# achraf-15/neural_image_compression

Measured on AMD Instinct MI355X. Metric: images/sec (256x256 RGB, batch 32) fwd+bwd, higher is better.
Workload: dtype f32; 1 GPU; cfg2: JointAutoregressiveHierarchical(M=192,K=1) fwd+rd_loss(lambda=0.01)+bwd+Adam, 32x3x256x256 per GPU, fp32; global_batch=32, parallelism=dp1, step=eager (autograd)

## Files before the change

### include/lic.h

```cpp
#ifndef LIC_H
#define LIC_H

#include <stddef.h>
#include <stdint.h>

#ifdef __cplusplus
extern "C" {
#endif

#define LIC_ABI_VERSION 4

typedef void* lic_stream_t;

enum lic_status {
  LIC_OK = 0,
  LIC_ERR_INVALID = -1,
  LIC_ERR_UNSUPPORTED = -2,
  LIC_ERR_LAUNCH = -3,
  LIC_ERR_WORKSPACE = -4
};

enum lic_epilogue {
  LIC_EPI_NONE = 0,
  LIC_EPI_LEAKY = 1,
// ... 256 lines not shown
                 double bias_correction2, lic_stream_t stream);

enum { LIC_REDUCE_SLABS = 0, LIC_REDUCE_COLUMNS = 1 };
enum { LIC_REDUCE_EPI_NONE = 0, LIC_REDUCE_EPI_REPARAM = 1 };
#define LIC_REDUCE_MAX_JOBS 32
typedef struct lic_reduce_job {
  const float* src;
  float* dst;
  const float* param;
  int64_t sm, smr, sn, snr, stap;
  int32_t kind, epilogue;
  int32_t splitk, ntaps, Cm, Cn, Mvalid, Nvalid, mdiv, ndiv;
  float scale, bound;
  int32_t block0, nblocks;
} lic_reduce_job;
int lic_wgrad_bf16_partial(const lic_wgrad_desc* d, void* workspace, size_t workspace_bytes, lic_reduce_job* job,
                           lic_stream_t stream);
int lic_colsum_bf16_partial(const void* in, int64_t ld, int64_t P, int32_t C, float scale, float* out, void* workspace,
                            size_t workspace_bytes, lic_reduce_job* job, lic_stream_t stream);
int lic_colsum2_bf16_partial(const void* in_a, const void* in_b, int64_t ld, int64_t P, int32_t C, float scale,
                             float* out_a, float* out_b, void* workspace, size_t workspace_bytes, lic_reduce_job* jobs2,
                             lic_stream_t stream);
int lic_leaky_bwd_colsum_bf16(const void* y, const void* dy, void* dx, int64_t P, int32_t C, float slope, float* out,
                              void* workspace, size_t workspace_bytes, lic_reduce_job* job, lic_stream_t stream);
int lic_reduce_batch(const lic_reduce_job* jobs, int32_t njobs, lic_stream_t stream);

int lic_head_convt_bf16_supported(int32_t Cin, int32_t Cout, int32_t kh, int32_t kw, int32_t stride, int32_t pad,
                                  int32_t out_pad);
int lic_head_convt_bf16(const void* x, const void* w_packed, const float* bias, float* out, int32_t B, int32_t Hi,
                        int32_t Wi, int32_t Cin, lic_stream_t stream);
int lic_stem_conv_bf16(const float* x, const void* w_packed, const float* bias, void* y, int32_t B, int32_t H, int32_t W,
                       int32_t Cout, lic_stream_t stream);

typedef struct lic_plan lic_plan;
int lic_plan_create(void* hip_graph, lic_plan** out);
int lic_plan_info(const lic_plan* plan, int64_t* info);
int lic_plan_replay(lic_plan* plan, lic_stream_t main, const lic_stream_t* sides, int32_t n_sides);
int lic_plan_tune(lic_plan* plan, lic_stream_t main, const lic_stream_t* sides, int32_t n_sides, double* result);
void lic_plan_destroy(lic_plan* plan);
const char* lic_plan_last_error(void);

int lic_version(void);
int lic_last_hip_error(void);
const char* lic_arch(void);

#ifdef __cplusplus
}
#endif
#endif
```

### neural_image_compression_amd/_lib.py

```python
from __future__ import annotations

import ctypes as C
import os

_HERE = os.path.dirname(os.path.abspath(__file__))
LIB_PATH = os.path.join(_HERE, "liblic_hip.so")

EPI_NONE, EPI_LEAKY, EPI_MUL_LEAKY_MASK, EPI_GDN, EPI_IGDN, EPI_GDN_BWD, EPI_IGDN_BWD, EPI_CONV_GDN, EPI_CONV_IGDN = range(9)
FE_NPARAM = 43

_vp, _i32, _i64, _f32, _sz = C.c_void_p, C.c_int32, C.c_int64, C.c_float, C.c_size_t


class IgemmDesc(C.Structure):
    _fields_ = [("in_", _vp), ("w", _vp), ("bias", _vp), ("out", _vp), ("out2", _vp), ("aux", _vp),
                ("aux2", _vp), ("aux3", _vp), ("res", _vp),
                ("in_ld", _i64), ("out_ld", _i64), ("out2_ld", _i64), ("aux_ld", _i64),
                ("aux2_ld", _i64), ("aux3_ld", _i64), ("res_ld", _i64),
                ("B", _i32), ("Hi", _i32), ("Wi", _i32), ("Cin", _i32),
                ("Ho", _i32), ("Wo", _i32), ("Cout", _i32),
                ("kh", _i32), ("kw", _i32), ("stride", _i32), ("pad", _i32),
                ("transposed", _i32), ("prologue", _i32), ("epilogue", _i32),
                ("tap_mask", C.c_uint32), ("slope", _f32), ("workspace", _vp), ("workspace_bytes", _sz),
                ("out3", _vp), ("out3_ld", _i64),
# ... 118 lines not shown
    "lic_gdn_bwd_bf16_partial_rows": (_i64, [_i64]),
    "lic_gdn_bwd_bf16": (C.c_int, [_vp, _vp, _vp, _vp, _vp, _vp, _vp, _vp, _i64, _i32, _i32, _vp]),
    "lic_gdn_bwd_bf16_recompute": (C.c_int, [_vp, _vp, _vp, _vp, _vp, _vp, _vp, _vp, _vp, _i64, _i32, _i32, _vp]),
    "lic_leaky_bwd_bf16": (C.c_int, [_vp, _vp, _vp, _i64, _f32, _vp]),
    "lic_leaky_bwd_colsum_bf16": (C.c_int, [_vp, _vp, _vp, _i64, _i32, _f32, _vp, _vp, _sz, C.POINTER(ReduceJob), _vp]),
    "lic_igemm_fused_gdn_supported": (C.c_int, [_i32, _i32]),
    "lic_igemm_fused_gdn_preferred": (C.c_int, [C.POINTER(IgemmDesc)]),
    "lic_gdn_supported": (C.c_int, [_i32]),
    "lic_gdn_fwd": (C.c_int, [_vp, _vp, _vp, _vp, _vp, _vp, _i64, _i32, _i32, _vp]),
    "lic_gdn_bwd_partial_rows": (_i64, [_i64]),
    "lic_gdn_bwd": (C.c_int, [_vp, _vp, _vp, _vp, _vp, _vp, _vp, _vp, _i64, _i32, _i32, _vp]),
    "lic_factorized_cdf_tables": (C.c_int, [_vp, _i32, _i32, _i32, _vp, _vp]),
    "lic_gmm_cdf_tables": (C.c_int, [_vp, _i64, _i32, _i32, _i32, _vp, _vp, _vp]),
    "lic_rans_decode_step": (C.c_int, [_vp] * 8 + [_i32] * 4 + [_vp, _vp, _i64, _vp]),
    "lic_rans_encode_pick": (C.c_int, [_vp] * 4 + [_i32, _i64, _i32, _i32] + [_vp] * 4),
    "lic_rans_encode": (C.c_int, [_vp] * 3 + [_i64, _i32, _i64, _vp, _i64, _vp, _vp, _vp]),
    "lic_msssim_workspace_bytes": (_sz, [_i32, _i32, _i32, _i32]),
    "lic_msssim": (C.c_int, [_vp, _vp, _i32, _i32, _i32, _i32, _i64, _i64, _i64, _i64, _f32, _vp, _vp, _vp, _sz,
                             _vp]),
    "lic_msssim_bwd_workspace_bytes": (_sz, [_i32, _i32, _i32, _i32]),
    "lic_msssim_bwd": (C.c_int, [_vp, _vp, _i32, _i32, _i32, _i32, _i64, _i64, _i64, _i64, _f32, _vp, _vp, _sz, _vp,
                                 _vp, _vp, _sz, _vp]),
    "lic_u8_to_f32": (C.c_int, [_vp, _vp, _i64, _vp]),
    "lic_window_u8_to_f32": (C.c_int, [_vp, _vp, _i32, _i32, _i32, _i32, _i32, _vp, _vp]),
    "lic_window_f32": (C.c_int, [_vp, _i64, _i64, _i64, _i64] + [_i32] * 9 + [_vp, _vp]),
    "lic_tensor_stats_workspace_bytes": (_sz, []),
    "lic_tensor_stats": (C.c_int, [_vp, _i64, _i32, _f32, _f32, _vp, _vp, _vp, _sz, _vp]),
    "lic_prep_plan": (_i64, [C.POINTER(PrepJob), _i32]),
    "lic_prep_run": (C.c_int, [_vp, _i32, _i64, _vp]),
    "lic_adam_plan": (_i64, [C.POINTER(AdamJob), _i32]),
    "lic_adam_run": (C.c_int, [_vp, _i32, _i64, _vp] + [C.c_double] * 7 + [_vp]),
    "lic_head_convt_bf16_supported": (C.c_int, [_i32] * 7),
    "lic_head_convt_bf16": (C.c_int, [_vp, _vp, _vp, _vp, _i32, _i32, _i32, _i32, _vp]),
    "lic_stem_conv_bf16": (C.c_int, [_vp, _vp, _vp, _vp, _i32, _i32, _i32, _i32, _vp]),
    "lic_plan_create": (C.c_int, [_vp, C.POINTER(C.c_void_p)]),
    "lic_plan_info": (C.c_int, [_vp, C.POINTER(C.c_int64)]),
    "lic_plan_replay": (C.c_int, [_vp, _vp, C.POINTER(C.c_void_p), _i32]),
    "lic_plan_tune": (C.c_int, [_vp, _vp, C.POINTER(C.c_void_p), _i32, C.POINTER(C.c_double)]),
    "lic_plan_destroy": (None, [_vp]),
    "lic_plan_last_error": (C.c_char_p, []),
    "lic_version": (C.c_int, []),
    "lic_last_hip_error": (C.c_int, []),
    "lic_arch": (C.c_char_p, []),
}

_lib = None


class LicError(RuntimeError):
    pass


def load():
    global _lib
    if _lib is None:
        if not os.path.exists(LIB_PATH):
            raise LicError(
                f"{LIB_PATH} not found: the HIP extension is not built. Run "
                "`python -c 'import __graft_entry__ as g; g.build()'` (or make -C "
                "neural_image_compression_amd/csrc). There is no CPU fallback.")
        lib = C.CDLL(LIB_PATH)
        for name, (res, args) in SIGNATURES.items():
            fn = getattr(lib, name)
            fn.restype = res
            fn.argtypes = args
        _lib = lib
    return _lib
# ... 10 lines not shown
```

### neural_image_compression_amd/functional.py

```python
from __future__ import annotations

import ctypes as C
from typing import Optional, Tuple

import torch

from . import _lib as L
from .reductions import can_defer, defer, flush_point, flush_reductions

PEDESTAL = float(2.0 ** -36)
LIKELIHOOD_BOUND = 1e-9

PROFILE = None
PROFILE_MIN_FLOP = 0.0
FORCE_IGEMM = None
FORCE_WGRAD = None
KERNEL_TRACE = None
GRAD_VIEWS = {}
PREPARED = {}
AUX_STREAM = None
PLAN_RECORDING = False


_raw_stream = getattr(torch._C, "_cuda_getCurrentRawStream", None)
# ... 332 lines not shown
    return _pack_conv_weight(weight.detach(), False, for_dgrad=False)


@torch.no_grad()
def conv2d_prepacked(x, w_packed, bias, cout, kernel, stride=1, padding=0, leaky=False, slope=0.01, tap_mask=0,
                     pin_tile=False):
    _require_cuda(x, w_packed, bias)
    xh = _nhwc(x)
    B, Hi, Wi, Cin = xh.shape
    Ho, Wo = conv_out_size(Hi, Wi, kernel, stride, padding, False)
    out = torch.empty((B, Ho, Wo, cout), device=x.device, dtype=torch.float32)
    global FORCE_IGEMM
    saved = FORCE_IGEMM
    if pin_tile and Cin % 4 == 0 and cout % 64 == 0:
        FORCE_IGEMM = (64, 1, 0)
    try:
        _igemm(xh, w_packed, out, B=B, Hi=Hi, Wi=Wi, Cin=Cin, Ho=Ho, Wo=Wo, Cout=cout, kh=kernel, kw=kernel,
               stride=stride, pad=padding, transposed=False, bias=bias,
               epilogue=L.EPI_LEAKY if leaky else L.EPI_NONE, slope=slope, tap_mask=tap_mask)
    finally:
        FORCE_IGEMM = saved
    return _nchw_view(out)


def conv_transpose2d(x, weight, bias, stride=1, padding=0, output_padding=0, leaky=False, slope=0.01,
                     residual=None):
    return _ConvFn.apply(x, weight, bias, stride, padding, output_padding, True, leaky, slope, 0, residual)


def _kpad(kh, kw, c):
    return (kh * kw * c + 3) // 4 * 4


def _image_conv_columns(xh, weight, stride, pad):
    B, Hi, Wi, Cin = xh.shape
    Cout, _, kh, kw = weight.shape
    Ho, Wo = conv_out_size(Hi, Wi, kh, stride, pad, False)
    Kp = _kpad(kh, kw, Cin)
    P = B * Ho * Wo
    col = torch.empty((P, Kp), device=xh.device, dtype=torch.float32)
    L.check(L.load().lic_im2col(_ptr(xh), _ptr(col), B, Hi, Wi, Cin, Ho, Wo, kh, kw, stride, pad, Kp,
                                _stream()), "lic_im2col")
    taps = kh * kw
    wpk = prepared(weight, "f32.stem")
    if wpk is None:
        wp = torch.zeros((Kp, Cout), device=xh.device, dtype=torch.float32)
        _permute3(weight.contiguous(), wp, (taps, Cin, Cout), (1, taps, Cin * taps), (Cin * Cout, Cout, 1))
        wpk = _pack_dense(wp)
    return col, wpk, Ho, Wo, Kp


def _image_conv_backward(col, weight, g, stride, pad, in_shape, need_dx, need_dw, need_db):
    B, Hi, Wi, Cin = in_shape
    _, Ho, Wo, Cout = g.shape
    _, _, kh, kw = weight.shape
    taps, Kp, P = kh * kw, col.shape[1], B * Ho * Wo
    lib = L.load()
    dx = dw = db = None
    if need_dx:
        wpT = torch.zeros((Cout, Kp), device=g.device, dtype=torch.float32)
        _permute3(weight.contiguous(), wpT, (Cout, Cin, taps), (Cin * taps, taps, 1), (Kp, 1, Cin))
        dcol = torch.empty((P, Kp), device=g.device, dtype=torch.float32)
        _igemm(g, _pack_dense(wpT), dcol, B=1, Hi=1, Wi=P, Cin=Cout, Ho=1, Wo=P, Cout=Kp, kh=1, kw=1, stride=1,
               pad=0, transposed=False)
        dxh = torch.empty((B, Hi, Wi, Cin), device=g.device, dtype=torch.float32)
        L.check(lib.lic_col2im(_ptr(dcol), None, _ptr(dxh), B, Ho, Wo, Cin, Hi, Wi, kh, kw, stride,
                               pad, Kp, _stream()), "lic_col2im")
        dx = _nchw_view(dxh)
    if need_dw:
        dw = grad_like(weight)
        tmp = torch.empty((Kp, Cout), device=g.device, dtype=torch.float32)
        _wgrad(col, g, tmp, B=1, Hs=1, Ws=P, Cp=Kp, Hl=1, Wl=P, Cg=Cout, kh=1, kw=1, stride=1, pad=0,
               g_is_row=False, dst_sm=Cout, dst_sn=1, dst_stap=0)
        _permute3(tmp, dw, (taps, Cin, Cout), (Cin * Cout, Cout, 1), (1, taps, Cin * taps))
    if need_db:
        db = _bias_grad(g, P, Cout)
    return dx, dw, db


class _ImageConvFn(torch.autograd.Function):

    @staticmethod
    def forward(ctx, x, weight, bias, stride, pad, leaky, slope):
        _require_cuda(x, weight, bias)
        xh = _nhwc(x)
        B = xh.shape[0]
        Cout = weight.shape[0]
        col, wp, Ho, Wo, Kp = _image_conv_columns(xh, weight, stride, pad)
        P = B * Ho * Wo
        out = torch.empty((B, Ho, Wo, Cout), device=x.device, dtype=torch.float32)
        _igemm(col, wp, out, B=1, Hi=1, Wi=P, Cin=Kp, Ho=1, Wo=P, Cout=Cout, kh=1, kw=1, stride=1,
               pad=0, transposed=False, bias=bias, epilogue=L.EPI_LEAKY if leaky else L.EPI_NONE,
               slope=slope)
        ctx.save_for_backward(col, weight, out if leaky else None)
        ctx.cfg = (stride, pad, leaky, slope, tuple(xh.shape), bias is not None)
        return _nchw_view(out)

    @staticmethod
    def backward(ctx, gy):
        col, weight, yh = ctx.saved_tensors
        stride, pad, leaky, slope, in_shape, has_bias = ctx.cfg
        g = _nhwc(gy)
        if leaky:
            g = _leaky_bwd(yh, g, slope)
        else:
            _carry_partial(gy, g)
        dx, dw, db = _image_conv_backward(col, weight, g, stride, pad, in_shape, ctx.needs_input_grad[0],
                                          ctx.needs_input_grad[1], has_bias and ctx.needs_input_grad[2])
        return dx, dw, db, None, None, None, None


class _ImageConvGDNFn(torch.autograd.Function):

    @staticmethod
    def forward(ctx, x, weight, bias, beta, gamma, stride, pad, inverse, beta_bound, gamma_bound, pedestal, keep=True):
        _require_cuda(x, weight, bias, beta, gamma)
        xh = _nhwc(x)
        B = xh.shape[0]
        Cout = weight.shape[0]
        col, wp, Ho, Wo, Kp = _image_conv_columns(xh, weight, stride, pad)
        P = B * Ho * Wo
        beta_e, gT = _gdn_operands(beta, gamma, beta_bound, gamma_bound, pedestal)
        y = torch.empty((B, Ho, Wo, Cout), device=x.device, dtype=torch.float32)
        conv_out = torch.empty_like(y) if keep else None
        norm = torch.empty_like(y) if keep else None
        _igemm(col, wp, y, B=1, Hi=1, Wi=P, Cin=Kp, Ho=1, Wo=P, Cout=Cout, kh=1, kw=1, stride=1,
               pad=0, transposed=False, bias=bias, epilogue=L.EPI_CONV_IGDN if inverse else L.EPI_CONV_GDN,
               out2=norm, out3=conv_out, aux=gT, aux2=beta_e)
        ctx.save_for_backward(col, weight, conv_out, norm, beta, gamma)
        ctx.cfg = (stride, pad, tuple(xh.shape), inverse, beta_bound, gamma_bound, bias is not None, pedestal)
        return _nchw_view(y)

    @staticmethod
    def backward(ctx, gy):
        col, weight, conv_out, norm, beta, gamma = ctx.saved_tensors
        stride, pad, in_shape, inverse, beta_bound, gamma_bound, has_bias, pedestal = ctx.cfg
        need = ctx.needs_input_grad
        g_conv, dbeta, dgamma = _gdn_backward(conv_out, norm, beta, gamma, _nhwc(gy), inverse,
                                              beta_bound, gamma_bound, pedestal, True, need[3], need[4])
        dx, dw, db = _image_conv_backward(col, weight, g_conv, stride, pad, in_shape, need[0], need[1],
                                          has_bias and need[2])
        return dx, dw, db, dbeta, dgamma, None, None, None, None, None, None, None


class _ImageConvTFn(torch.autograd.Function):

    @staticmethod
    def forward(ctx, x, weight, bias, stride, pad, out_pad):
        _require_cuda(x, weight, bias)
        xh = _nhwc(x)
        B, Hi, Wi, Cin = xh.shape
        _, Cout, kh, kw = weight.shape
        Ho, Wo = conv_out_size(Hi, Wi, kh, stride, pad, True, out_pad)
        taps, Kp, P = kh * kw, _kpad(kh, kw, Cout), B * Hi * Wi
        lib = L.load()
        wpk = prepared(weight, "f32.head")
        if wpk is None:
            wp = torch.zeros((Cin, Kp), device=x.device, dtype=torch.float32)
            _permute3(weight.contiguous(), wp, (Cin, Cout, taps), (Cout * taps, taps, 1), (Kp, 1, Cout))
            wpk = _pack_dense(wp)
        col = torch.empty((P, Kp), device=x.device, dtype=torch.float32)
        _igemm(xh, wpk, col, B=1, Hi=1, Wi=P, Cin=Cin, Ho=1, Wo=P, Cout=Kp, kh=1, kw=1, stride=1, pad=0,
               transposed=False)
        out = torch.empty((B, Ho, Wo, Cout), device=x.device, dtype=torch.float32)
        L.check(lib.lic_col2im(_ptr(col), _ptr(bias), _ptr(out), B, Hi, Wi, Cout, Ho, Wo, kh, kw, stride,
                               pad, Kp, _stream()), "lic_col2im")
        ctx.save_for_backward(xh, weight)
        ctx.cfg = (stride, pad, (Ho, Wo), bias is not None)
        return _nchw_view(out)

    @staticmethod
    def backward(ctx, gy):
        xh, weight = ctx.saved_tensors
        stride, pad, (Ho, Wo), has_bias = ctx.cfg
        g = _nhwc(gy)
        B, Hi, Wi, Cin = xh.shape
        _, Cout, kh, kw = weight.shape
        taps, Kp, P = kh * kw, _kpad(kh, kw, Cout), B * Hi * Wi
        lib = L.load()
        dcol = torch.empty((P, Kp), device=g.device, dtype=torch.float32)
        L.check(lib.lic_im2col(_ptr(g), _ptr(dcol), B, Ho, Wo, Cout, Hi, Wi, kh, kw, stride, pad, Kp,
                               _stream()), "lic_im2col")
        dx = dw = db = None
        if ctx.needs_input_grad[0]:
            wpk = prepared(weight, "f32.head_dx")
            if wpk is None:
                wpT = torch.zeros((Kp, Cin), device=g.device, dtype=torch.float32)
                _permute3(weight.contiguous(), wpT, (taps, Cout, Cin), (1, taps, Cout * taps),
                          (Cout * Cin, Cin, 1))
                wpk = _pack_dense(wpT)
            dxh = torch.empty_like(xh)
            _igemm(dcol, wpk, dxh, B=1, Hi=1, Wi=P, Cin=Kp, Ho=1, Wo=P, Cout=Cin, kh=1, kw=1, stride=1,
                   pad=0, transposed=False)
            dx = _nchw_view(dxh)
        if ctx.needs_input_grad[1]:
            dw = grad_like(weight)
            tmp = torch.empty((Cin, Kp), device=g.device, dtype=torch.float32)
            _wgrad(xh, dcol, tmp, B=1, Hs=1, Ws=P, Cp=Cin, Hl=1, Wl=P, Cg=Kp, kh=1, kw=1, stride=1, pad=0,
                   g_is_row=True, dst_sm=1, dst_sn=Kp, dst_stap=0)
            _permute3(tmp, dw, (Cin, taps, Cout), (Kp, Cout, 1), (Cout * taps, 1, taps))
        if has_bias and ctx.needs_input_grad[2]:
            db = _colsum(g, B * Ho * Wo, Cout)
        return dx, dw, db, None, None, None


def image_conv2d(x, weight, bias, stride, padding, leaky=False, slope=0.01):
    return _ImageConvFn.apply(x, weight, bias, stride, padding, leaky, slope)


def image_conv_transpose2d(x, weight, bias, stride, padding, output_padding):
    return _ImageConvTFn.apply(x, weight, bias, stride, padding, output_padding)


class _LeakyFn(torch.autograd.Function):
    @staticmethod
    def forward(ctx, x, slope):
        _require_cuda(x)
        xc = x.contiguous()
        y = _leaky_bwd(xc, xc, slope)
        ctx.save_for_backward(y)
        ctx.slope = slope
        return y

    @staticmethod
    def backward(ctx, gy):
        (y,) = ctx.saved_tensors
        return _leaky_bwd(y, gy.contiguous(), ctx.slope), None


def leaky_relu(x, slope=0.01):
    return _LeakyFn.apply(x, slope)


class _GDNFn(torch.autograd.Function):
    @staticmethod
    def forward(ctx, x, beta, gamma, inverse, beta_bound, gamma_bound, pedestal, res, keep=True):
# ... 562 lines not shown
```

Measured before the change: 1433 images/s.

## Add fused f32 MFMA kernel for the 3-channel transposed-conv image head

Adds a direct HIP kernel for the stride-2 5x5 transposed convolution that produces the RGB output. Each block computes a halo tile's per-tap partial products with f32 MFMA into shared memory, then gathers them into output pixels with the bias added. This replaces the igemm into a padded column buffer followed by a separate col2im pass, so the large intermediate column tensor is no longer written and re-read. Only the forward path changes; the backward still uses the existing col-based route, and the shape restrictions fall back to the old path otherwise.

```diff
diff --git a/include/lic.h b/include/lic.h
--- a/include/lic.h
+++ b/include/lic.h
@@ -312,6 +312,11 @@
 int lic_stem_conv_bf16(const float* x, const void* w_packed, const float* bias, void* y, int32_t B, int32_t H, int32_t W,
                        int32_t Cout, lic_stream_t stream);
 
+int lic_head_convt_f32_supported(int32_t Cin, int32_t Cout, int32_t kh, int32_t kw, int32_t stride, int32_t pad,
+                                 int32_t out_pad);
+int lic_head_convt_f32(const float* x, const float* w, const float* bias, float* out, int32_t B, int32_t Hi, int32_t Wi,
+                       int32_t Cin, lic_stream_t stream);
+
 typedef struct lic_plan lic_plan;
 int lic_plan_create(void* hip_graph, lic_plan** out);
 int lic_plan_info(const lic_plan* plan, int64_t* info);
diff --git a/neural_image_compression_amd/_lib.py b/neural_image_compression_amd/_lib.py
--- a/neural_image_compression_amd/_lib.py
+++ b/neural_image_compression_amd/_lib.py
@@ -174,6 +174,8 @@
     "lic_adam_run": (C.c_int, [_vp, _i32, _i64, _vp] + [C.c_double] * 7 + [_vp]),
     "lic_head_convt_bf16_supported": (C.c_int, [_i32] * 7),
     "lic_head_convt_bf16": (C.c_int, [_vp, _vp, _vp, _vp, _i32, _i32, _i32, _i32, _vp]),
+    "lic_head_convt_f32_supported": (C.c_int, [_i32] * 7),
+    "lic_head_convt_f32": (C.c_int, [_vp, _vp, _vp, _vp, _i32, _i32, _i32, _i32, _vp]),
     "lic_stem_conv_bf16": (C.c_int, [_vp, _vp, _vp, _vp, _i32, _i32, _i32, _i32, _vp]),
     "lic_plan_create": (C.c_int, [_vp, C.POINTER(C.c_void_p)]),
     "lic_plan_info": (C.c_int, [_vp, C.POINTER(C.c_int64)]),
diff --git a/neural_image_compression_amd/csrc/lic_head_f32.hip b/neural_image_compression_amd/csrc/lic_head_f32.hip
--- /dev/null
+++ b/neural_image_compression_amd/csrc/lic_head_f32.hip
@@ -0,0 +1,172 @@
+#include "lic_common.h"
+
+namespace {
+
+constexpr int HF_TH = 8, HF_TW = 16;
+constexpr int HF_HR = HF_TH + 2, HF_HC = HF_TW + 2;
+constexpr int HF_HP = HF_HR * HF_HC;
+constexpr int HF_PT = 3;
+constexpr int HF_LD = 84;
+constexpr int HF_NT = 5;
+static_assert(4 * HF_PT * 16 >= HF_HP, "the four waves cover the halo block");
+
+struct HeadF32Params {
+  const float* x;
+  const float* w;
+  const float* bias;
+  float* out;
+  int B, Hi, Wi, tiles_x, tiles_y;
+  long ntiles;
+};
+
+template <int NC>
+__global__ __launch_bounds__(256) void head_convt_f32_kernel(const HeadF32Params p) {
+  constexpr int C = 16 * NC, WLD = C + 4;
+  __shared__ __attribute__((aligned(16))) float wl[16 * HF_NT * WLD];
+  __shared__ __attribute__((aligned(16))) float col[4 * HF_PT * 16 * HF_LD];
+  const int tid = threadIdx.x, lane = tid & 63, l16 = lane & 15, g = lane >> 4;
+  const int wave = __builtin_amdgcn_readfirstlane(tid >> 6);
+  for (int i = tid; i < 5 * WLD; i += 256) wl[75 * WLD + i] = 0.0f;
+  for (int i = tid; i < C * 75; i += 256) {
+    const int ci = i / 75, r = i - ci * 75, co = r / 25, tap = r - co * 25;
+    wl[(3 * tap + co) * WLD + ci] = p.w[i];
+  }
+  float bs[3] = {0.f, 0.f, 0.f};
+  if (p.bias)
+#pragma unroll
+    for (int c = 0; c < 3; ++c) bs[c] = p.bias[c];
+  const int Ho = 2 * p.Hi, Wo = 2 * p.Wi;
+  __syncthreads();
+
+  for (long tile = blockIdx.x; tile < p.ntiles; tile += gridDim.x) {
+    const int tx = (int)(tile % p.tiles_x);
+    const long rest = tile / p.tiles_x;
+    const int ty = (int)(rest % p.tiles_y), b = (int)(rest / p.tiles_y);
+    const int y0 = ty * HF_TH, x0 = tx * HF_TW;
+    const float* src[HF_PT];
+    bool ok[HF_PT];
+#pragma unroll
+    for (int i = 0; i < HF_PT; ++i) {
+      const int hp = (wave * HF_PT + i) * 16 + l16;
+      const int hr = hp / HF_HC, hc = hp - hr * HF_HC;
+      const int iy = y0 - 1 + hr, ix = x0 - 1 + hc;
+      ok[i] = hp < HF_HP && iy >= 0 && iy < p.Hi && ix >= 0 && ix < p.Wi;
+      src[i] = p.x + (((long)b * p.Hi + (ok[i] ? iy : 0)) * p.Wi + (ok[i] ? ix : 0)) * C + 4 * g;
+    }
+    f32x4 acc[HF_PT][HF_NT];
+#pragma unroll
+    for (int i = 0; i < HF_PT; ++i)
+#pragma unroll
+      for (int t = 0; t < HF_NT; ++t) acc[i][t] = f32x4{0.f, 0.f, 0.f, 0.f};
+    f32x4 xq[HF_PT], xn[HF_PT];
+#pragma unroll
+    for (int i = 0; i < HF_PT; ++i) xq[i] = *reinterpret_cast<const f32x4*>(src[i]);
+#pragma unroll
+    for (int c = 0; c < NC; ++c) {
+      if (c + 1 < NC)
+#pragma unroll
+        for (int i = 0; i < HF_PT; ++i) xn[i] = *reinterpret_cast<const f32x4*>(src[i] + 16 * (c + 1));
+      f32x4 wf[HF_NT];
+#pragma unroll
+      for (int t = 0; t < HF_NT; ++t) wf[t] = *reinterpret_cast<const f32x4*>(wl + (16 * t + l16) * WLD + 16 * c + 4 * g);
+#pragma unroll
+      for (int i = 0; i < HF_PT; ++i)
+        if (!ok[i]) xq[i] = f32x4{0.f, 0.f, 0.f, 0.f};
+#pragma unroll
+      for (int e = 0; e < 4; ++e)
+#pragma unroll
+        for (int t = 0; t < HF_NT; ++t)
+#pragma unroll
+          for (int i = 0; i < HF_PT; ++i)
+            acc[i][t] = __builtin_amdgcn_mfma_f32_16x16x4f32(wf[t][e], xq[i][e], acc[i][t], 0, 0, 0);
+#pragma unroll
+      for (int i = 0; i < HF_PT; ++i) xq[i] = xn[i];
+    }
+#pragma unroll
+    for (int i = 0; i < HF_PT; ++i) {
+      float* row = col + ((wave * HF_PT + i) * 16 + l16) * HF_LD + 4 * g;
+#pragma unroll
+      for (int t = 0; t < HF_NT; ++t) *reinterpret_cast<f32x4*>(row + 16 * t) = acc[i][t];
+    }
+    __syncthreads();
+#pragma unroll
+    for (int h = 0; h < 2; ++h) {
+      const int oyl = (tid >> 5) + 8 * h, oxl = tid & 31;
+      const int qy = oyl >> 1, py = oyl & 1, qx = oxl >> 1, px = oxl & 1;
+      float o0 = bs[0], o1 = bs[1], o2 = bs[2];
+#pragma unroll
+      for (int a = 0; a < 3; ++a) {
+        const int ky = py + 2 * a;
+        if (ky > 4) continue;
+        const int hr = qy + 2 - a;
+#pragma unroll
+        for (int bb = 0; bb < 3; ++bb) {
+          const int kx = px + 2 * bb;
+          if (kx > 4) continue;
+          const int hc = qx + 2 - bb;
+          const float* c3 = col + (hr * HF_HC + hc) * HF_LD + 3 * (5 * ky + kx);
+          o0 += c3[0];
+          o1 += c3[1];
+          o2 += c3[2];
+        }
+      }
+      const int oy = 2 * y0 + oyl, ox = 2 * x0 + oxl;
+      if (oy < Ho && ox < Wo) {
+        float* dst = p.out + (((long)b * Ho + oy) * Wo + ox) * 3;
+        dst[0] = o0;
+        dst[1] = o1;
+        dst[2] = o2;
+      }
+    }
+    __syncthreads();
+  }
+}
+
+template <int NC>
+int head_f32_launch(const HeadF32Params& p, hipStream_t s) {
+  static const int slots = [] {
+    int per_cu = 0, cus = 0, devid = 0;
+    if (hipOccupancyMaxActiveBlocksPerMultiprocessor(&per_cu, (const void*)head_convt_f32_kernel<NC>, 256, 0) != hipSuccess || per_cu < 1)
+      per_cu = 1;
+    if (hipGetDevice(&devid) != hipSuccess ||
+        hipDeviceGetAttribute(&cus, hipDeviceAttributeMultiprocessorCount, devid) != hipSuccess || cus < 1)
+      cus = 256;
+    return per_cu * cus;
+  }();
+  long grid = p.ntiles < slots ? p.ntiles : slots;
+  const long rounds = (p.ntiles + grid - 1) / grid;
+  grid = (p.ntiles + rounds - 1) / rounds;
+  hipLaunchKernelGGL((head_convt_f32_kernel<NC>), dim3((unsigned)grid), dim3(256), 0, s, p);
+  return lic_check_launch();
+}
+
+}
+
+LIC_EXPORT int lic_head_convt_f32_supported(int32_t Cin, int32_t Cout, int32_t kh, int32_t kw, int32_t stride, int32_t pad,
+                                            int32_t out_pad) {
+  return (Cin == 64 || Cin == 128 || Cin == 192) && Cout == 3 && kh == 5 && kw == 5 && stride == 2 && pad == 2 && out_pad == 1;
+}
+
+LIC_EXPORT int lic_head_convt_f32(const float* x, const float* w, const float* bias, float* out, int32_t B, int32_t Hi,
+                                  int32_t Wi, int32_t Cin, lic_stream_t stream) {
+  if (!x || !w || !out || B <= 0 || Hi <= 0 || Wi <= 0) return LIC_ERR_INVALID;
+  if (!(Cin == 64 || Cin == 128 || Cin == 192)) return LIC_ERR_UNSUPPORTED;
+  if ((reinterpret_cast<uintptr_t>(x) & 15) || (reinterpret_cast<uintptr_t>(w) & 3) || (reinterpret_cast<uintptr_t>(out) & 3))
+    return LIC_ERR_INVALID;
+  HeadF32Params p;
+  p.x = x;
+  p.w = w;
+  p.bias = bias;
+  p.out = out;
+  p.B = B;
+  p.Hi = Hi;
+  p.Wi = Wi;
+  p.tiles_x = (Wi + HF_TW - 1) / HF_TW;
+  p.tiles_y = (Hi + HF_TH - 1) / HF_TH;
+  p.ntiles = (long)B * p.tiles_x * p.tiles_y;
+  if ((long)B * Hi * Wi * Cin > 0x7FFFFFFFFFL) return LIC_ERR_UNSUPPORTED;
+  hipStream_t s = (hipStream_t)stream;
+  if (Cin == 64) return head_f32_launch<4>(p, s);
+  if (Cin == 128) return head_f32_launch<8>(p, s);
+  return head_f32_launch<12>(p, s);
+}
diff --git a/neural_image_compression_amd/functional.py b/neural_image_compression_amd/functional.py
--- a/neural_image_compression_amd/functional.py
+++ b/neural_image_compression_amd/functional.py
@@ -510,6 +510,17 @@
         Ho, Wo = conv_out_size(Hi, Wi, kh, stride, pad, True, out_pad)
         taps, Kp, P = kh * kw, _kpad(kh, kw, Cout), B * Hi * Wi
         lib = L.load()
+        if head_direct_supported(Cin, Cout, kh, kw, stride, pad, out_pad):
+            out = torch.empty((B, Ho, Wo, Cout), device=x.device, dtype=torch.float32)
+            wc = weight.contiguous()
+            name = f"head_convt_f32_kernel<{Cin // 16}>"
+            _trace(name)
+            _timed(name, 2.0 * P * Cin * taps * Cout, 4 * (P * Cin + B * Ho * Wo * Cout),
+                   lambda: L.check(lib.lic_head_convt_f32(_ptr(xh), _ptr(wc), _ptr(bias), _ptr(out), B, Hi, Wi, Cin,
+                                                          _stream()), "lic_head_convt_f32"))
+            ctx.save_for_backward(xh, weight)
+            ctx.cfg = (stride, pad, (Ho, Wo), bias is not None)
+            return _nchw_view(out)
         wpk = prepared(weight, "f32.head")
         if wpk is None:
             wp = torch.zeros((Cin, Kp), device=x.device, dtype=torch.float32)
@@ -558,6 +569,10 @@
         if has_bias and ctx.needs_input_grad[2]:
             db = _colsum(g, B * Ho * Wo, Cout)
         return dx, dw, db, None, None, None
+
+
+def head_direct_supported(Cin, Cout, kh, kw, stride, pad, out_pad) -> bool:
+    return bool(L.load().lic_head_convt_f32_supported(Cin, Cout, kh, kw, stride, pad, out_pad))
 
 
 def image_conv2d(x, weight, bias, stride, padding, leaky=False, slope=0.01):
```

Result: no change. 1439 images/s, median of 6 (+0.4%).

## Add direct fp32 RGB stem/head conv kernels avoiding im2col/col2im buffers

Applied to the files above, without the earlier changes.

Adds HIP kernels for the 5x5 stride-2 RGB convolutions: a transposed-conv head that computes per-tile columns in LDS and scatters them directly, a stem-style conv for its input gradient, and a patch weight-gradient kernel that builds image patches in LDS. These replace the large materialised im2col/col2im column buffers and their separate GEMMs. The image-conv forward now saves the raw input instead of the column matrix for backward. This cuts global memory traffic and buffer allocation, but adds fixed-shape kernels and a split-K slab reduction.

```diff
diff --git a/include/lic.h b/include/lic.h
--- a/include/lic.h
+++ b/include/lic.h
@@ -312,6 +312,15 @@
 int lic_stem_conv_bf16(const float* x, const void* w_packed, const float* bias, void* y, int32_t B, int32_t H, int32_t W,
                        int32_t Cout, lic_stream_t stream);
 
+int lic_rgb_f32_supported(int32_t C, int32_t Crgb, int32_t kh, int32_t kw, int32_t stride, int32_t pad);
+int lic_head_convt_f32(const float* x, const float* w_packed, const float* bias, float* out, int32_t B, int32_t Hi,
+                       int32_t Wi, int32_t Cin, lic_stream_t stream);
+int lic_stem_conv_f32(const float* x, const float* w_packed, float* y, int32_t B, int32_t H, int32_t W, int32_t Cout,
+                      lic_stream_t stream);
+size_t lic_patch_wgrad_f32_workspace_bytes(int32_t B, int32_t H, int32_t W, int32_t C);
+int lic_patch_wgrad_f32(const float* img, const float* act, float* dst, int32_t B, int32_t H, int32_t W, int32_t C,
+                        int64_t dst_sm, int64_t dst_sn, void* workspace, size_t workspace_bytes, lic_stream_t stream);
+
 typedef struct lic_plan lic_plan;
 int lic_plan_create(void* hip_graph, lic_plan** out);
 int lic_plan_info(const lic_plan* plan, int64_t* info);
diff --git a/neural_image_compression_amd/_lib.py b/neural_image_compression_amd/_lib.py
--- a/neural_image_compression_amd/_lib.py
+++ b/neural_image_compression_amd/_lib.py
@@ -175,6 +175,11 @@
     "lic_head_convt_bf16_supported": (C.c_int, [_i32] * 7),
     "lic_head_convt_bf16": (C.c_int, [_vp, _vp, _vp, _vp, _i32, _i32, _i32, _i32, _vp]),
     "lic_stem_conv_bf16": (C.c_int, [_vp, _vp, _vp, _vp, _i32, _i32, _i32, _i32, _vp]),
+    "lic_rgb_f32_supported": (C.c_int, [_i32] * 6),
+    "lic_head_convt_f32": (C.c_int, [_vp, _vp, _vp, _vp, _i32, _i32, _i32, _i32, _vp]),
+    "lic_stem_conv_f32": (C.c_int, [_vp, _vp, _vp, _i32, _i32, _i32, _i32, _vp]),
+    "lic_patch_wgrad_f32_workspace_bytes": (_sz, [_i32] * 4),
+    "lic_patch_wgrad_f32": (C.c_int, [_vp, _vp, _vp, _i32, _i32, _i32, _i32, _i64, _i64, _vp, _sz, _vp]),
     "lic_plan_create": (C.c_int, [_vp, C.POINTER(C.c_void_p)]),
     "lic_plan_info": (C.c_int, [_vp, C.POINTER(C.c_int64)]),
     "lic_plan_replay": (C.c_int, [_vp, _vp, C.POINTER(C.c_void_p), _i32]),
diff --git a/neural_image_compression_amd/csrc/lic_rgb_f32.hip b/neural_image_compression_amd/csrc/lic_rgb_f32.hip
--- /dev/null
+++ b/neural_image_compression_amd/csrc/lic_rgb_f32.hip
@@ -0,0 +1,440 @@
+#include "lic_common.h"
+#include "lic_conv_plan.h"
+
+namespace {
+
+constexpr int RG_TH = 8, RG_TW = 16;
+constexpr int RG_HR = RG_TH + 2, RG_HC = RG_TW + 2;
+constexpr int RG_HP = RG_HR * RG_HC;
+constexpr int RG_MT = (RG_HP + 15) / 16;
+constexpr int RG_LD = 84;
+constexpr int RG_IR = 2 * RG_TH + 3, RG_IC = 2 * RG_TW + 3;
+constexpr int RG_IMG = RG_IR * RG_IC * 3;
+constexpr int RG_K = 75, RG_KP = 76, RG_KT = 5;
+
+__device__ __forceinline__ long rg_pk(int k, int n, int ntile) {
+  const int cb = k >> 4, r = k & 15;
+  return ((((long)cb * ntile + (n >> 5)) * 2 + ((r >> 2) & 1)) * 64 + ((r >> 3) << 5) + (n & 31)) * 4 + (r & 3);
+}
+
+__device__ __forceinline__ void rg_panel_to_lds(const float* __restrict__ w, float* lds, int K4, int N, int ntile) {
+  for (int i = threadIdx.x; i < K4 * N; i += 256) {
+    const int k4 = i / N, n = i - k4 * N;
+    *reinterpret_cast<f32x4*>(lds + 4 * i) = *reinterpret_cast<const f32x4*>(w + rg_pk(4 * k4, n, ntile));
+  }
+}
+
+__device__ __forceinline__ void rg_image_to_lds(const float* __restrict__ img, float* lds, int b, int H, int W, int y0, int x0) {
+  for (int i = threadIdx.x; i < RG_IMG; i += 256) {
+    const int r = i / (RG_IC * 3), c3 = i - r * (RG_IC * 3);
+    const int iy = 2 * y0 - 2 + r, ix = 2 * x0 - 2 + c3 / 3;
+    float v = 0.0f;
+    if (iy >= 0 && iy < H && ix >= 0 && ix < W) v = img[(((long)b * H + iy) * W + ix) * 3 + (c3 % 3)];
+    lds[i] = v;
+  }
+}
+
+__device__ __forceinline__ int rg_col_ofs(int kc) {
+  const int tap = kc / 3, co = kc - 3 * tap;
+  const int ky = tap / 5, kx = tap - 5 * ky;
+  return (ky * RG_IC + kx) * 3 + co;
+}
+
+struct TileGeom {
+  int tiles_x, tiles_y;
+  long ntiles;
+};
+
+struct HeadParams {
+  const float* x;
+  const float* w;
+  const float* bias;
+  float* out;
+  int B, Hi, Wi;
+  TileGeom g;
+};
+
+template <int NC>
+__global__ __launch_bounds__(256, 1) void head_convt_f32_kernel(const HeadParams p) {
+  constexpr int C = 16 * NC;
+  __shared__ __attribute__((aligned(16))) float wl[C * 80];
+  __shared__ __attribute__((aligned(16))) float col[RG_MT * 16 * RG_LD];
+  const int tid = threadIdx.x, lane = tid & 63, li = lane & 15, kq = lane >> 4;
+  const int wave = __builtin_amdgcn_readfirstlane(tid >> 6);
+  rg_panel_to_lds(p.w, wl, C / 4, 80, 4);
+  float bs[3] = {0.f, 0.f, 0.f};
+  if (p.bias)
+#pragma unroll
+    for (int c = 0; c < 3; ++c) bs[c] = p.bias[c];
+  const int Ho = 2 * p.Hi, Wo = 2 * p.Wi;
+  __syncthreads();
+
+  for (long tile = blockIdx.x; tile < p.g.ntiles; tile += gridDim.x) {
+    const int tx = (int)(tile % p.g.tiles_x);
+    const long rest = tile / p.g.tiles_x;
+    const int ty = (int)(rest % p.g.tiles_y), b = (int)(rest / p.g.tiles_y);
+    const int y0 = ty * RG_TH, x0 = tx * RG_TW;
+    f32x4 xq[2][NC];
+    auto load = [&](int m, f32x4* dst) {
+      const int hp = m * 16 + li;
+      const int hr = hp / RG_HC, hc = hp - hr * RG_HC;
+      const int iy = y0 - 1 + hr, ix = x0 - 1 + hc;
+      const bool ok = hp < RG_HP && iy >= 0 && iy < p.Hi && ix >= 0 && ix < p.Wi;
+      const float* src = p.x + (((long)b * p.Hi + (ok ? iy : 0)) * p.Wi + (ok ? ix : 0)) * C + 4 * kq;
+#pragma unroll
+      for (int q = 0; q < NC; ++q) dst[q] = *reinterpret_cast<const f32x4*>(src + 16 * q);
+      if (!ok)
+#pragma unroll
+        for (int q = 0; q < NC; ++q) dst[q] = f32x4{0.f, 0.f, 0.f, 0.f};
+    };
+    load(wave, xq[0]);
+#pragma unroll
+    for (int it = 0; it < RG_MT / 4; ++it) {
+      const int m = wave + 4 * it;
+      if (it + 1 < RG_MT / 4) load(m + 4, xq[(it + 1) & 1]);
+      const f32x4* xv = xq[it & 1];
+      f32x4 acc[RG_KT];
+#pragma unroll
+      for (int t = 0; t < RG_KT; ++t) acc[t] = f32x4{0.f, 0.f, 0.f, 0.f};
+#pragma unroll
+      for (int q = 0; q < NC; ++q) {
+#pragma unroll
+        for (int t = 0; t < RG_KT; ++t) {
+          const f32x4 wv = *reinterpret_cast<const f32x4*>(wl + ((q * 4 + kq) * 80 + 16 * t + li) * 4);
+#pragma unroll
+          for (int j = 0; j < 4; ++j) acc[t] = __builtin_amdgcn_mfma_f32_16x16x4f32(wv[j], xv[q][j], acc[t], 0, 0, 0);
+        }
+      }
+      float* row = col + (m * 16 + li) * RG_LD + 4 * kq;
+#pragma unroll
+      for (int t = 0; t < RG_KT; ++t) *reinterpret_cast<f32x4*>(row + 16 * t) = acc[t];
+    }
+    __syncthreads();
+#pragma unroll
+    for (int h = 0; h < 2; ++h) {
+      const int oyl = (tid >> 5) + 8 * h, oxl = tid & 31;
+      const int qy = oyl >> 1, py = oyl & 1, qx = oxl >> 1, px = oxl & 1;
+      float o0 = bs[0], o1 = bs[1], o2 = bs[2];
+#pragma unroll
+      for (int a = 0; a < 3; ++a) {
+        const int ky = py + 2 * a;
+        if (ky > 4) continue;
+        const int hr = qy + 2 - a;
+#pragma unroll
+        for (int bb = 0; bb < 3; ++bb) {
+          const int kx = px + 2 * bb;
+          if (kx > 4) continue;
+          const int hc = qx + 2 - bb;
+          const float* c3 = col + (hr * RG_HC + hc) * RG_LD + 3 * (5 * ky + kx);
+          o0 += c3[0];
+          o1 += c3[1];
+          o2 += c3[2];
+        }
+      }
+      const int oy = 2 * y0 + oyl, ox = 2 * x0 + oxl;
+      if (oy < Ho && ox < Wo) {
+        float* dst = p.out + (((long)b * Ho + oy) * Wo + ox) * 3;
+        dst[0] = o0;
+        dst[1] = o1;
+        dst[2] = o2;
+      }
+    }
+    __syncthreads();
+  }
+}
+
+struct StemParams {
+  const float* x;
+  const float* w;
+  float* y;
+  int B, H, W, Hy, Wy;
+  TileGeom g;
+};
+
+template <int NC>
+__global__ __launch_bounds__(256, 2) void stem_conv_f32_kernel(const StemParams p) {
+  constexpr int C = 16 * NC;
+  __shared__ __attribute__((aligned(16))) float wl[80 * C];
+  __shared__ float img[RG_IMG];
+  const int tid = threadIdx.x, lane = tid & 63, li = lane & 15, kq = lane >> 4;
+  const int wave = __builtin_amdgcn_readfirstlane(tid >> 6);
+  rg_panel_to_lds(p.w, wl, 20, C, C / 32);
+  int ofs[RG_KT][4];
+#pragma unroll
+  for (int q = 0; q < RG_KT; ++q)
+#pragma unroll
+    for (int j = 0; j < 4; ++j) {
+      const int k = 16 * q + 4 * kq + j;
+      ofs[q][j] = k < RG_K ? rg_col_ofs(k) : -1;
+    }
+
+  for (long tile = blockIdx.x; tile < p.g.ntiles; tile += gridDim.x) {
+    const int tx = (int)(tile % p.g.tiles_x);
+    const long rest = tile / p.g.tiles_x;
+    const int ty = (int)(rest % p.g.tiles_y), b = (int)(rest / p.g.tiles_y);
+    const int y0 = ty * RG_TH, x0 = tx * RG_TW;
+    __syncthreads();
+    rg_image_to_lds(p.x, img, b, p.H, p.W, y0, x0);
+    __syncthreads();
+    float pv[2][RG_KT][4];
+#pragma unroll
+    for (int r = 0; r < 2; ++r) {
+      const int corner = ((2 * (2 * wave + r)) * RG_IC + 2 * li) * 3;
+#pragma unroll
+      for (int q = 0; q < RG_KT; ++q)
+#pragma unroll
+        for (int j = 0; j < 4; ++j) pv[r][q][j] = ofs[q][j] >= 0 ? img[corner + ofs[q][j]] : 0.0f;
+    }
+    const int ox = x0 + li;
+    float* dst[2];
+    bool ok[2];
+#pragma unroll
+    for (int r = 0; r < 2; ++r) {
+      const int oy = y0 + 2 * wave + r;
+      ok[r] = oy < p.Hy && ox < p.Wy;
+      dst[r] = p.y + (((long)b * p.Hy + (ok[r] ? oy : 0)) * p.Wy + (ok[r] ? ox : 0)) * C + 4 * kq;
+    }
+#pragma unroll
+    for (int t = 0; t < NC; ++t) {
+      f32x4 acc[2] = {f32x4{0.f, 0.f, 0.f, 0.f}, f32x4{0.f, 0.f, 0.f, 0.f}};
+#pragma unroll
+      for (int q = 0; q < RG_KT; ++q) {
+        const f32x4 wv = *reinterpret_cast<const f32x4*>(wl + ((q * 4 + kq) * C + 16 * t + li) * 4);
+#pragma unroll
+        for (int j = 0; j < 4; ++j)
+#pragma unroll
+          for (int r = 0; r < 2; ++r) acc[r] = __builtin_amdgcn_mfma_f32_16x16x4f32(wv[j], pv[r][q][j], acc[r], 0, 0, 0);
+      }
+#pragma unroll
+      for (int r = 0; r < 2; ++r)
+        if (ok[r]) *reinterpret_cast<f32x4*>(dst[r] + 16 * t) = acc[r];
+    }
+  }
+}
+
+struct PatchWgradParams {
+  const float* img;
+  const float* act;
+  float* slabs;
+  int B, H, W, Hy, Wy;
+  int tiles_per_split;
+  TileGeom g;
+};
+
+template <int NC>
+__global__ __launch_bounds__(256, 2) void patch_wgrad_f32_kernel(const PatchWgradParams p) {
+  constexpr int C = 16 * NC, NW = NC / 4;
+  __shared__ float img[RG_IMG];
+  const int tid = threadIdx.x, lane = tid & 63, li = lane & 15, kq = lane >> 4;
+  const int wave = __builtin_amdgcn_readfirstlane(tid >> 6);
+  int ofs[RG_KT];
+#pragma unroll
+  for (int mt = 0; mt < RG_KT; ++mt) ofs[mt] = 16 * mt + li < RG_K ? rg_col_ofs(16 * mt + li) : -1;
+  f32x4 acc[RG_KT][NW];
+#pragma unroll
+  for (int mt = 0; mt < RG_KT; ++mt)
+#pragma unroll
+    for (int i = 0; i < NW; ++i) acc[mt][i] = f32x4{0.f, 0.f, 0.f, 0.f};
+  const int ch = 16 * NW * wave + li;
+
+  const long t0 = (long)blockIdx.x * p.tiles_per_split;
+  const long t1 = t0 + p.tiles_per_split < p.g.ntiles ? t0 + p.tiles_per_split : p.g.ntiles;
+  for (long tile = t0; tile < t1; ++tile) {
+    const int tx = (int)(tile % p.g.tiles_x);
+    const long rest = tile / p.g.tiles_x;
+    const int ty = (int)(rest % p.g.tiles_y), b = (int)(rest / p.g.tiles_y);
+    const int y0 = ty * RG_TH, x0 = tx * RG_TW;
+    __syncthreads();
+    rg_image_to_lds(p.img, img, b, p.H, p.W, y0, x0);
+    __syncthreads();
+#pragma unroll
+    for (int s8 = 0; s8 < 4; ++s8) {
+      float bv[8][NW];
+#pragma unroll
+      for (int u = 0; u < 8; ++u) {
+        const int s = 8 * s8 + u;
+        const int oy = y0 + (s >> 2), ox = x0 + 4 * (s & 3) + kq;
+        const bool ok = oy < p.Hy && ox < p.Wy;
+        const float* src = p.act + (((long)b * p.Hy + (ok ? oy : 0)) * p.Wy + (ok ? ox : 0)) * C + ch;
+#pragma unroll
+        for (int i = 0; i < NW; ++i) {
+          const float v = src[16 * i];
+          bv[u][i] = ok ? v : 0.0f;
+        }
+      }
+#pragma unroll
+      for (int u = 0; u < 8; ++u) {
+        const int s = 8 * s8 + u;
+        const int corner = ((2 * (s >> 2)) * RG_IC + 2 * (4 * (s & 3) + kq)) * 3;
+#pragma unroll
+        for (int mt = 0; mt < RG_KT; ++mt) {
+          const float av = ofs[mt] >= 0 ? img[corner + ofs[mt]] : 0.0f;
+#pragma unroll
+          for (int i = 0; i < NW; ++i) acc[mt][i] = __builtin_amdgcn_mfma_f32_16x16x4f32(av, bv[u][i], acc[mt][i], 0, 0, 0);
+        }
+      }
+    }
+  }
+  float* slab = p.slabs + (long)blockIdx.x * RG_KP * C;
+#pragma unroll
+  for (int mt = 0; mt < RG_KT; ++mt)
+#pragma unroll
+    for (int j = 0; j < 4; ++j) {
+      const int m = 16 * mt + 4 * kq + j;
+      if (m < RG_KP)
+#pragma unroll
+        for (int i = 0; i < NW; ++i) slab[(long)m * C + ch + 16 * i] = acc[mt][i][j];
+    }
+}
+
+bool rg_al16(const void* q) { return (reinterpret_cast<uintptr_t>(q) & 15) == 0; }
+bool rg_c_ok(int C) { return C == 64 || C == 128 || C == 192; }
+
+TileGeom rg_tiles(int B, int Hy, int Wy) {
+  TileGeom g;
+  g.tiles_x = (Wy + RG_TW - 1) / RG_TW;
+  g.tiles_y = (Hy + RG_TH - 1) / RG_TH;
+  g.ntiles = (long)B * g.tiles_x * g.tiles_y;
+  return g;
+}
+
+template <typename K>
+int rg_slots(K kernel) {
+  int per_cu = 0, cus = 0, devid = 0;
+  if (hipOccupancyMaxActiveBlocksPerMultiprocessor(&per_cu, (const void*)kernel, 256, 0) != hipSuccess || per_cu < 1) per_cu = 1;
+  if (hipGetDevice(&devid) != hipSuccess ||
+      hipDeviceGetAttribute(&cus, hipDeviceAttributeMultiprocessorCount, devid) != hipSuccess || cus < 1)
+    cus = 256;
+  return per_cu * cus;
+}
+
+template <int NC>
+int head_launch(const HeadParams& p, hipStream_t s) {
+  static const int slots = rg_slots(head_convt_f32_kernel<NC>);
+  const long grid = p.g.ntiles < slots ? p.g.ntiles : slots;
+  hipLaunchKernelGGL((head_convt_f32_kernel<NC>), dim3((unsigned)grid), dim3(256), 0, s, p);
+  return lic_check_launch();
+}
+
+template <int NC>
+int stem_launch(const StemParams& p, hipStream_t s) {
+  static const int slots = rg_slots(stem_conv_f32_kernel<NC>);
+  const long grid = p.g.ntiles < slots ? p.g.ntiles : slots;
+  hipLaunchKernelGGL((stem_conv_f32_kernel<NC>), dim3((unsigned)grid), dim3(256), 0, s, p);
+  return lic_check_launch();
+}
+
+template <int NC>
+int pwg_slots() {
+  static const int slots = rg_slots(patch_wgrad_f32_kernel<NC>);
+  return slots;
+}
+
+int pwg_splits(const TileGeom& g, int C, int* tiles_per_split) {
+  const int slots = C == 64 ? pwg_slots<4>() : C == 128 ? pwg_slots<8>() : pwg_slots<12>();
+  long sk = lic_pick_splits(1, slots, g.ntiles);
+  if (sk > g.ntiles) sk = g.ntiles;
+  if (sk < 1) sk = 1;
+  const long tps = (g.ntiles + sk - 1) / sk;
+  *tiles_per_split = (int)tps;
+  return (int)((g.ntiles + tps - 1) / tps);
+}
+
+}
+
+LIC_EXPORT int lic_rgb_f32_supported(int32_t C, int32_t Crgb, int32_t kh, int32_t kw, int32_t stride, int32_t pad) {
+  return rg_c_ok(C) && Crgb == 3 && kh == 5 && kw == 5 && stride == 2 && pad == 2;
+}
+
+LIC_EXPORT int lic_head_convt_f32(const float* x, const float* w_packed, const float* bias, float* out, int32_t B, int32_t Hi,
+                                  int32_t Wi, int32_t Cin, lic_stream_t stream) {
+  if (!x || !w_packed || !out || B <= 0 || Hi <= 0 || Wi <= 0) return LIC_ERR_INVALID;
+  if (!rg_c_ok(Cin)) return LIC_ERR_UNSUPPORTED;
+  if (!rg_al16(x) || !rg_al16(w_packed) || (reinterpret_cast<uintptr_t>(out) & 3)) return LIC_ERR_INVALID;
+  if ((long)B * Hi * Wi > 0x7FFFFFFFL / 16) return LIC_ERR_UNSUPPORTED;
+  HeadParams p;
+  p.x = x;
+  p.w = w_packed;
+  p.bias = bias;
+  p.out = out;
+  p.B = B;
+  p.Hi = Hi;
+  p.Wi = Wi;
+  p.g = rg_tiles(B, Hi, Wi);
+  hipStream_t s = (hipStream_t)stream;
+  if (Cin == 64) return head_launch<4>(p, s);
+  if (Cin == 128) return head_launch<8>(p, s);
+  return head_launch<12>(p, s);
+}
+
+LIC_EXPORT int lic_stem_conv_f32(const float* x, const float* w_packed, float* y, int32_t B, int32_t H, int32_t W, int32_t Cout,
+                                 lic_stream_t stream) {
+  if (!x || !w_packed || !y || B <= 0 || H <= 0 || W <= 0) return LIC_ERR_INVALID;
+  if (!rg_c_ok(Cout)) return LIC_ERR_UNSUPPORTED;
+  if (!rg_al16(y) || !rg_al16(w_packed) || (reinterpret_cast<uintptr_t>(x) & 3)) return LIC_ERR_INVALID;
+  if ((long)B * H * W > 0x7FFFFFFFL / 16) return LIC_ERR_UNSUPPORTED;
+  StemParams p;
+  p.x = x;
+  p.w = w_packed;
+  p.y = y;
+  p.B = B;
+  p.H = H;
+  p.W = W;
+  p.Hy = (H + 1) / 2;
+  p.Wy = (W + 1) / 2;
+  p.g = rg_tiles(B, p.Hy, p.Wy);
+  hipStream_t s = (hipStream_t)stream;
+  if (Cout == 64) return stem_launch<4>(p, s);
+  if (Cout == 128) return stem_launch<8>(p, s);
+  return stem_launch<12>(p, s);
+}
+
+LIC_EXPORT size_t lic_patch_wgrad_f32_workspace_bytes(int32_t B, int32_t H, int32_t W, int32_t C) {
+  if (B <= 0 || H <= 0 || W <= 0 || !rg_c_ok(C)) return 0;
+  int tps = 0;
+  const int sk = pwg_splits(rg_tiles(B, (H + 1) / 2, (W + 1) / 2), C, &tps);
+  return (size_t)sk * RG_KP * C * sizeof(float);
+}
+
+LIC_EXPORT int lic_patch_wgrad_f32(const float* img, const float* act, float* dst, int32_t B, int32_t H, int32_t W, int32_t C,
+                                   int64_t dst_sm, int64_t dst_sn, void* workspace, size_t workspace_bytes,
+                                   lic_stream_t stream) {
+  if (!img || !act || !dst || !workspace || B <= 0 || H <= 0 || W <= 0) return LIC_ERR_INVALID;
+  if (!rg_c_ok(C)) return LIC_ERR_UNSUPPORTED;
+  if ((reinterpret_cast<uintptr_t>(img) & 3) || (reinterpret_cast<uintptr_t>(act) & 3) || !rg_al16(workspace)) return LIC_ERR_INVALID;
+  if ((long)B * H * W > 0x7FFFFFFFL / 16) return LIC_ERR_UNSUPPORTED;
+  PatchWgradParams p;
+  p.img = img;
+  p.act = act;
+  p.slabs = (float*)workspace;
+  p.B = B;
+  p.H = H;
+  p.W = W;
+  p.Hy = (H + 1) / 2;
+  p.Wy = (W + 1) / 2;
+  p.g = rg_tiles(B, p.Hy, p.Wy);
+  const int sk = pwg_splits(p.g, C, &p.tiles_per_split);
+  if (workspace_bytes < (size_t)sk * RG_KP * C * sizeof(float)) return LIC_ERR_WORKSPACE;
+  hipStream_t s = (hipStream_t)stream;
+  if (C == 64)
+    hipLaunchKernelGGL((patch_wgrad_f32_kernel<4>), dim3(sk), dim3(256), 0, s, p);
+  else if (C == 128)
+    hipLaunchKernelGGL((patch_wgrad_f32_kernel<8>), dim3(sk), dim3(256), 0, s, p);
+  else
+    hipLaunchKernelGGL((patch_wgrad_f32_kernel<12>), dim3(sk), dim3(256), 0, s, p);
+  int rc = lic_check_launch();
+  if (rc != LIC_OK) return rc;
+  lic_reduce_job job = {};
+  job.src = p.slabs;
+  job.dst = dst;
+  job.sm = dst_sm;
+  job.sn = dst_sn;
+  job.kind = LIC_REDUCE_SLABS;
+  job.epilogue = LIC_REDUCE_EPI_NONE;
+  job.splitk = sk;
+  job.ntaps = 1;
+  job.Cm = RG_KP;
+  job.Cn = C;
+  job.scale = 1.0f;
+  return lic_reduce_batch(&job, 1, stream);
+}
diff --git a/neural_image_compression_amd/functional.py b/neural_image_compression_amd/functional.py
--- a/neural_image_compression_amd/functional.py
+++ b/neural_image_compression_amd/functional.py
@@ -388,6 +388,25 @@
     return (kh * kw * c + 3) // 4 * 4
 
 
+RGB_DIRECT = True
+
+
+def _rgb_direct(C, Crgb, kh, kw, stride, pad, *aligned):
+    return (RGB_DIRECT and all(t.data_ptr() % 16 == 0 for t in aligned)
+            and bool(L.load().lic_rgb_f32_supported(C, Crgb, kh, kw, stride, pad)))
+
+
+def _patch_wgrad(img, act, dst, C, dst_sm, dst_sn):
+    lib = L.load()
+    B, H, W, _ = img.shape
+    nbytes = lib.lic_patch_wgrad_f32_workspace_bytes(B, H, W, C)
+    ws = torch.empty((max(nbytes, 4) + 3) // 4, device=img.device, dtype=torch.float32)
+    P = act.shape[0] * act.shape[1] * act.shape[2]
+    _timed(f"patch_wgrad_f32_kernel<{C // 16}>", 2.0 * P * 75 * C, 4 * (P * C + B * H * W * 3),
+           lambda: L.check(lib.lic_patch_wgrad_f32(_ptr(img), _ptr(act), _ptr(dst), B, H, W, C, dst_sm, dst_sn, _ptr(ws), nbytes,
+                                                   _stream()), "lic_patch_wgrad_f32"))
+
+
 def _image_conv_columns(xh, weight, stride, pad):
     B, Hi, Wi, Cin = xh.shape
     Cout, _, kh, kw = weight.shape
@@ -410,7 +429,7 @@
     B, Hi, Wi, Cin = in_shape
     _, Ho, Wo, Cout = g.shape
     _, _, kh, kw = weight.shape
-    taps, Kp, P = kh * kw, col.shape[1], B * Ho * Wo
+    taps, Kp, P = kh * kw, _kpad(kh, kw, Cin), B * Ho * Wo
     lib = L.load()
     dx = dw = db = None
     if need_dx:
@@ -426,8 +445,11 @@
     if need_dw:
         dw = grad_like(weight)
         tmp = torch.empty((Kp, Cout), device=g.device, dtype=torch.float32)
-        _wgrad(col, g, tmp, B=1, Hs=1, Ws=P, Cp=Kp, Hl=1, Wl=P, Cg=Cout, kh=1, kw=1, stride=1, pad=0,
-               g_is_row=False, dst_sm=Cout, dst_sn=1, dst_stap=0)
+        if col.dim() == 4:
+            _patch_wgrad(col, g, tmp, Cout, Cout, 1)
+        else:
+            _wgrad(col, g, tmp, B=1, Hs=1, Ws=P, Cp=Kp, Hl=1, Wl=P, Cg=Cout, kh=1, kw=1, stride=1, pad=0,
+                   g_is_row=False, dst_sm=Cout, dst_sn=1, dst_stap=0)
         _permute3(tmp, dw, (taps, Cin, Cout), (Cin * Cout, Cout, 1), (1, taps, Cin * taps))
     if need_db:
         db = _bias_grad(g, P, Cout)
@@ -448,7 +470,8 @@
         _igemm(col, wp, out, B=1, Hi=1, Wi=P, Cin=Kp, Ho=1, Wo=P, Cout=Cout, kh=1, kw=1, stride=1,
                pad=0, transposed=False, bias=bias, epilogue=L.EPI_LEAKY if leaky else L.EPI_NONE,
                slope=slope)
-        ctx.save_for_backward(col, weight, out if leaky else None)
+        keep_x = _rgb_direct(Cout, xh.shape[3], weight.shape[2], weight.shape[3], stride, pad)
+        ctx.save_for_backward(xh if keep_x else col, weight, out if leaky else None)
         ctx.cfg = (stride, pad, leaky, slope, tuple(xh.shape), bias is not None)
         return _nchw_view(out)
 
@@ -483,7 +506,8 @@
         _igemm(col, wp, y, B=1, Hi=1, Wi=P, Cin=Kp, Ho=1, Wo=P, Cout=Cout, kh=1, kw=1, stride=1,
                pad=0, transposed=False, bias=bias, epilogue=L.EPI_CONV_IGDN if inverse else L.EPI_CONV_GDN,
                out2=norm, out3=conv_out, aux=gT, aux2=beta_e)
-        ctx.save_for_backward(col, weight, conv_out, norm, beta, gamma)
+        keep_x = _rgb_direct(Cout, xh.shape[3], weight.shape[2], weight.shape[3], stride, pad)
+        ctx.save_for_backward(xh if keep_x else col, weight, conv_out, norm, beta, gamma)
         ctx.cfg = (stride, pad, tuple(xh.shape), inverse, beta_bound, gamma_bound, bias is not None, pedestal)
         return _nchw_view(y)
 
@@ -515,45 +539,61 @@
             wp = torch.zeros((Cin, Kp), device=x.device, dtype=torch.float32)
             _permute3(weight.contiguous(), wp, (Cin, Cout, taps), (Cout * taps, taps, 1), (Kp, 1, Cout))
             wpk = _pack_dense(wp)
-        col = torch.empty((P, Kp), device=x.device, dtype=torch.float32)
-        _igemm(xh, wpk, col, B=1, Hi=1, Wi=P, Cin=Cin, Ho=1, Wo=P, Cout=Kp, kh=1, kw=1, stride=1, pad=0,
-               transposed=False)
         out = torch.empty((B, Ho, Wo, Cout), device=x.device, dtype=torch.float32)
-        L.check(lib.lic_col2im(_ptr(col), _ptr(bias), _ptr(out), B, Hi, Wi, Cout, Ho, Wo, kh, kw, stride,
-                               pad, Kp, _stream()), "lic_col2im")
+        direct = out_pad == 1 and _rgb_direct(Cin, Cout, kh, kw, stride, pad, xh, wpk)
+        if direct:
+            _timed(f"head_convt_f32_kernel<{Cin // 16}>", 2.0 * P * Cin * taps * Cout, 4 * (P * Cin + B * Ho * Wo * Cout),
+                   lambda: L.check(lib.lic_head_convt_f32(_ptr(xh), _ptr(wpk), _ptr(bias), _ptr(out), B, Hi, Wi, Cin,
+                                                          _stream()), "lic_head_convt_f32"))
+        else:
+            col = torch.empty((P, Kp), device=x.device, dtype=torch.float32)
+            _igemm(xh, wpk, col, B=1, Hi=1, Wi=P, Cin=Cin, Ho=1, Wo=P, Cout=Kp, kh=1, kw=1, stride=1, pad=0,
+                   transposed=False)
+            L.check(lib.lic_col2im(_ptr(col), _ptr(bias), _ptr(out), B, Hi, Wi, Cout, Ho, Wo, kh, kw, stride,
+                                   pad, Kp, _stream()), "lic_col2im")
         ctx.save_for_backward(xh, weight)
-        ctx.cfg = (stride, pad, (Ho, Wo), bias is not None)
+        ctx.cfg = (stride, pad, (Ho, Wo), bias is not None, direct)
         return _nchw_view(out)
 
     @staticmethod
     def backward(ctx, gy):
         xh, weight = ctx.saved_tensors
-        stride, pad, (Ho, Wo), has_bias = ctx.cfg
+        stride, pad, (Ho, Wo), has_bias, direct = ctx.cfg
         g = _nhwc(gy)
         B, Hi, Wi, Cin = xh.shape
         _, Cout, kh, kw = weight.shape
         taps, Kp, P = kh * kw, _kpad(kh, kw, Cout), B * Hi * Wi
         lib = L.load()
-        dcol = torch.empty((P, Kp), device=g.device, dtype=torch.float32)
-        L.check(lib.lic_im2col(_ptr(g), _ptr(dcol), B, Ho, Wo, Cout, Hi, Wi, kh, kw, stride, pad, Kp,
-                               _stream()), "lic_im2col")
+        dcol = None
+        if not direct:
+            dcol = torch.empty((P, Kp), device=g.device, dtype=torch.float32)
+            L.check(lib.lic_im2col(_ptr(g), _ptr(dcol), B, Ho, Wo, Cout, Hi, Wi, kh, kw, stride, pad, Kp,
+                                   _stream()), "lic_im2col")
         dx = dw = db = None
         if ctx.needs_input_grad[0]:
             wpk = prepared(weight, "f32.head_dx")
-            if wpk is None:
+            if wpk is None or (direct and wpk.data_ptr() % 16):
                 wpT = torch.zeros((Kp, Cin), device=g.device, dtype=torch.float32)
                 _permute3(weight.contiguous(), wpT, (taps, Cout, Cin), (1, taps, Cout * taps),
                           (Cout * Cin, Cin, 1))
                 wpk = _pack_dense(wpT)
             dxh = torch.empty_like(xh)
-            _igemm(dcol, wpk, dxh, B=1, Hi=1, Wi=P, Cin=Kp, Ho=1, Wo=P, Cout=Cin, kh=1, kw=1, stride=1,
-                   pad=0, transposed=False)
+            if direct:
+                _timed(f"stem_conv_f32_kernel<{Cin // 16}>", 2.0 * P * Cin * taps * Cout, 4 * (P * Cin + B * Ho * Wo * Cout),
+                       lambda: L.check(lib.lic_stem_conv_f32(_ptr(g), _ptr(wpk), _ptr(dxh), B, Ho, Wo, Cin, _stream()),
+                                       "lic_stem_conv_f32"))
+            else:
+                _igemm(dcol, wpk, dxh, B=1, Hi=1, Wi=P, Cin=Kp, Ho=1, Wo=P, Cout=Cin, kh=1, kw=1, stride=1,
+                       pad=0, transposed=False)
             dx = _nchw_view(dxh)
         if ctx.needs_input_grad[1]:
             dw = grad_like(weight)
             tmp = torch.empty((Cin, Kp), device=g.device, dtype=torch.float32)
-            _wgrad(xh, dcol, tmp, B=1, Hs=1, Ws=P, Cp=Cin, Hl=1, Wl=P, Cg=Kp, kh=1, kw=1, stride=1, pad=0,
-                   g_is_row=True, dst_sm=1, dst_sn=Kp, dst_stap=0)
+            if direct:
+                _patch_wgrad(g, xh, tmp, Cin, 1, Kp)
+            else:
+                _wgrad(xh, dcol, tmp, B=1, Hs=1, Ws=P, Cp=Cin, Hl=1, Wl=P, Cg=Kp, kh=1, kw=1, stride=1, pad=0,
+                       g_is_row=True, dst_sm=1, dst_sn=Kp, dst_stap=0)
             _permute3(tmp, dw, (Cin, taps, Cout), (Kp, Cout, 1), (Cout * taps, 1, taps))
         if has_bias and ctx.needs_input_grad[2]:
             db = _colsum(g, B * Ho * Wo, Cout)
```

New measurement: 1442 images/s before, 1441 images/s after. Within noise of the previous version (-0.1%).
